# JanSpindler/NRC-HPM-Renderer

Hardware: AMD Instinct MI355X
Metric: Msamples/s + ms/frame at 1080p, 256^3 cloud (NRC path) (higher is better)
Workload: dtype f16 (fp16 MFMA operands, fp32 accumulate; fp32 integrator)

## Files before the change

nrc-hpm-renderer_amd/csrc/nrc_api.hip:

```cpp
#include <algorithm>
#include <array>
#include <chrono>
#include <cmath>
#include <cstdio>
#include <cstdlib>
#include <cstring>
#include <fstream>
#include <map>
#include <memory>
#include <mutex>
#include <random>
#include <string>
#include <thread>
#include <unordered_map>
#include <vector>

#include <dlfcn.h>
#include <rccl/rccl.h>

#include "nrc_integrator.hpp"
#include "nrc_mlp.hpp"
#include "nrc_checkpoint.hpp"
#include "nrc_occupancy.hpp"
#include "nrc_schedule.hpp"
// ... 317 lines not shown
    {
        if (owner_ == who) owner_ = nullptr;
        last_loss_event_ = nullptr;
    }

    void infer_all(const uint32_t* filter, hipStream_t s, bool skip_zero = false, const CompositeArgs* composite = nullptr,
                   const uint32_t* live_list = nullptr, const uint32_t* live_count = nullptr, hipEvent_t done = nullptr)
    {
        if (!initialised_) throw std::logic_error("SkyRenderer ERROR: InferAndTrain before Init");
        struct Tail {
            hipEvent_t e; hipStream_t s; bool armed = false;
            ~Tail() { if (armed) { try { finish_launch_tail(s); } catch (...) { launch_tail() = LaunchTail{}; } } else if (e) (void)hipEventRecord(e, s); }
        } tail{done, s};
        const bool one = infer_batches_.size() == 1;
        size_t last_batch = infer_batches_.size();
        for (size_t i = 0; i < infer_batches_.size(); i++)
            if (filter == nullptr || filter[i] != 0) last_batch = i;
        if (!one && filter == nullptr && live_list != nullptr && composite == nullptr && skip_zero && mlp_->encodes_in_kernel()) {
            if (done) { arm_launch_tail(done); tail.armed = true; }
            mlp_->infer(d_infer_in_, d_infer_out_, infer_count_, true, s, skip_zero, nullptr, live_list, live_count);
            return;
        }
        for (size_t i = 0; i < infer_batches_.size(); i++) {
            if (filter != nullptr && filter[i] == 0) continue;
            const auto& b = infer_batches_[i];
            if (done && i == last_batch) { arm_launch_tail(done); tail.armed = true; }
            CompositeArgs ca;
            if (composite) { ca = *composite; ca.q_base = b.first; }
            mlp_->infer(d_infer_in_ + (size_t)b.first * 5, d_infer_out_ + (size_t)b.first * 3, b.second, true, s, skip_zero, composite ? &ca : nullptr,
                        one ? live_list : nullptr, one ? live_count : nullptr);
        }
    }
    bool model_has_grid() const { return mlp_->has_grid(); }
    bool encodes_in_kernel() const { return mlp_->encodes_in_kernel(); }
    bool can_pre_encode(const void* who) const { return initialised_ && mlp_->can_pre_encode() && owner_ == who && owner_frames_ >= 2; }
    void pre_encode(const float* d_train_in, int parity, hipStream_t s)
    {
        pre_features_ = mlp_->pre_encode(d_train_in, train_batch_count_ * train_batch_size_, parity, s);
        pre_source_ = d_train_in;
    }
    bool wants_live_list() const { return infer_batches_.size() == 1 || mlp_->encodes_in_kernel(); }
    bool can_composite() const { return mlp_->can_composite(); }

    void train_all(hipStream_t st, hipEvent_t ev_infer_prev, hipEvent_t ev_infer_cur = nullptr, hipEvent_t done = nullptr)
    {
        if (!initialised_) throw std::logic_error("SkyRenderer ERROR: InferAndTrain before Init");
        poll_comm();
        for (uint32_t b = 0; b < train_batch_count_; b++) {
            const size_t o = (size_t)b * train_batch_size_;
            const bool vector_read = hook_ != nullptr || (comm_ != nullptr && !sparse_grid_);
            if (pre_source_ != d_train_in_) pre_features_ = nullptr;
            const void* ready = pre_features_ != nullptr ? (const void*)((const char*)pre_features_ + o * mlp_->enc_dims() * 2) : nullptr;
            mlp_->backward(d_train_in_ + o * 5, d_train_target_ + o * 3, train_batch_size_,
                           train_batch_size_ * loss_norm_factor_, st, vector_read, ready);
            if (comm_ || hook_) mlp_->guard_stale();
            if (comm_ && sparse_grid_) exchange_sparse(st);
            else if (comm_ && exchange_half_) exchange_half(st, mlp_->n_params());
            else if (comm_) Rccl::get().check(Rccl::get().all_reduce(mlp_->grad_ptr(), mlp_->grad_ptr(), (size_t)mlp_->n_params() + 2, ncclFloat,
                                                               ncclSum, comm_, st), "ncclAllReduce");
            if (hook_) {
                if (exchange_half_) round_grad_half(st, mlp_->n_params());
                hook_(hook_user_, mlp_->grad_ptr(), mlp_->n_params(), mlp_->loss_ptr(), (void*)st);
                if (exchange_half_) round_grad_half(st, mlp_->n_params(), true);
            }
            if (vector_read) mlp_->grad_vector_is_source();
            if (b == 0 && ev_infer_prev) NRC_HIP(hipStreamWaitEvent(st, ev_infer_prev, 0));
            if (b == 1 && ev_infer_cur) NRC_HIP(hipStreamWaitEvent(st, ev_infer_cur, 0));
            loss_pushed_++;
            const bool last = b + 1 == train_batch_count_;
            hipEvent_t after = (last && done) ? done : ev_loss_;
            LaunchTailScope tail(st, after);
            const bool published = mlp_->optimizer_step(st, loss_pushed_, d_loss_cell_);
            if (!published) {
                launch_last(k_publish_loss, dim3(1), dim3(1), 0u, st, (const float*)mlp_->loss_ptr(), loss_pushed_, d_loss_cell_);
                NRC_HIP(hipGetLastError());
            }
            tail.finish();
            last_loss_event_ = after;
        }
        if (train_batch_count_ == 0 && done) NRC_HIP(hipEventRecord(done, st));
        pre_features_ = nullptr;
    }

    void ensure_grid_lists(uint32_t n_lists)
    {
        const uint32_t cap = mlp_->grid_list_capacity(train_batch_size_);
        if (cap == grid_cap_ && n_lists <= grid_lists_) return;
        NRC_HIP(hipDeviceSynchronize());
        if (d_grid_send_) dev_free(d_grid_send_);
        if (d_grid_recv_) dev_free(d_grid_recv_);
        grid_cap_ = cap;
        grid_lists_ = n_lists;
        dev_alloc(&d_grid_send_, Mlp::grid_list_words(cap) * 4, "d_grid_send_");
        dev_alloc(&d_grid_recv_, Mlp::grid_list_words(cap) * 4 * n_lists, "d_grid_recv_");
    }
    void exchange_half(hipStream_t st, uint32_t n)
    {
        Rccl& r = Rccl::get();
        if (!r.group_start || !r.group_end) fail("librccl lacks ncclGroupStart / ncclGroupEnd");
        start_exchange_half(st, n);
        RcclGroup group(r);
        r.check(r.all_reduce(d_grad_half_, d_grad_half_, n, ncclHalf, ncclSum, comm_, st), "ncclAllReduce");
        r.check(r.all_reduce(mlp_->loss_ptr(), mlp_->loss_ptr(), 2, ncclFloat, ncclSum, comm_, st), "ncclAllReduce");
        group.end();
        finish_exchange_half(st, n);
    }
    void start_exchange_half(hipStream_t st, uint32_t n)
// ... 2417 lines not shown
```

nrc-hpm-renderer_amd/csrc/nrc_mlp.hip:

```cpp
#include "nrc_mlp.hpp"

#include <algorithm>
#include <cmath>
#include <cstdio>
#include <cstdlib>
#include <cstring>
#include <type_traits>

namespace nrc {

using half_t = _Float16;
using half8 = _Float16 __attribute__((ext_vector_type(8)));
using f32x16 = float __attribute__((ext_vector_type(16)));

namespace {

constexpr int ENC = 80;
constexpr int WIDTH = 64;
constexpr int KS0 = ENC / 16;
constexpr int KSH = WIDTH / 16;
constexpr int MT = WIDTH / 32;

__host__ __device__ inline int fmap80(int s, int h, int j)
{
// ... 1872 lines not shown
        }                                                                                                          \
    }
    NRC_WG_LOAD(a0, b0, 0)
    for (int s = 0; s < ksteps; s += 2 * U) {
        NRC_WG_LOAD(a1, b1, s + U)
        NRC_WG_MMA(a0, b0, s)
        NRC_WG_LOAD(a0, b0, s + 2 * U)
        NRC_WG_MMA(a1, b1, s + U)
    }
#undef NRC_WG_LOAD
#undef NRC_WG_MMA
#pragma unroll
    for (int t = 0; t < NTL; t++) {
        float* o = slab + T.param_off + 32u * (uint32_t)t + (uint32_t)r;
#pragma unroll
        for (int reg = 0; reg < 16; reg++) {
            const uint32_t row = (reg & 3) + 8 * (reg >> 2) + 4 * h;
            if (row < T.m_valid && bv[t]) o[(size_t)row * T.in_dim] = acc[t][reg];
        }
    }
}
#ifndef NRC_WGRAD2_MIN_WAVES
#define NRC_WGRAD2_MIN_WAVES 2
#endif
__global__ __launch_bounds__(WGRAD2_WAVES * 64, NRC_WGRAD2_MIN_WAVES) void k_wgrad2(const half_t* __restrict__ deltas, const half_t* __restrict__ acts, uint32_t n,
                                                             uint32_t chunk, uint32_t rows_d, uint32_t rows_a,
                                                             const WgradTask* __restrict__ tasks, int n_tasks, float* __restrict__ slabs,
                                                             uint32_t n_params)
{
    NRC_RAISE_WAVE_PRIORITY(1);
    const int lane = threadIdx.x & 63, wave = threadIdx.x >> 6;
    const int task = __builtin_amdgcn_readfirstlane((int)blockIdx.y * WGRAD2_WAVES + wave);
    if (task >= n_tasks) return;
    const WgradTask T = tasks[task];
    const uint32_t k0 = blockIdx.x * chunk;
    const uint32_t left = n - k0;
    const int ksteps = (int)((left < chunk ? left : chunk) >> 4);
    float* slab = slabs + (size_t)blockIdx.x * n_params;
    if constexpr (WGRAD2_NTL == 1) {
        wgrad_task<1>(T, deltas, acts, k0, ksteps, rows_d, rows_a, slab, lane);
    } else if constexpr (WGRAD2_NTL == 2) {
        if (T.n_tiles == 1) wgrad_task<1>(T, deltas, acts, k0, ksteps, rows_d, rows_a, slab, lane);
        else wgrad_task<2>(T, deltas, acts, k0, ksteps, rows_d, rows_a, slab, lane);
    } else {
        switch (T.n_tiles) {
        case 1: wgrad_task<1>(T, deltas, acts, k0, ksteps, rows_d, rows_a, slab, lane); break;
        case 2: wgrad_task<2>(T, deltas, acts, k0, ksteps, rows_d, rows_a, slab, lane); break;
        case 3: wgrad_task<3>(T, deltas, acts, k0, ksteps, rows_d, rows_a, slab, lane); break;
        default: wgrad_task<4>(T, deltas, acts, k0, ksteps, rows_d, rows_a, slab, lane); break;
        }
    }
}

template <class... Guard>
__global__ __launch_bounds__(256) void k_reduce_grads(const float* __restrict__ slabs, uint32_t n_chunks, uint32_t n_params,
                                                     float* __restrict__ grad, const float* __restrict__ loss_part,
                                                     uint32_t n_loss, float* __restrict__ loss, Guard... ga)
{
    NRC_RAISE_WAVE_PRIORITY(1);
    __shared__ float part[4][64];
    __shared__ float red[256];
    const uint32_t p = threadIdx.x & 63u, g = threadIdx.x >> 6;
    const uint32_t i = blockIdx.x * 64u + p;
    const uint32_t per = (n_chunks + 3u) / 4u;
    const uint32_t c0 = g * per, c1 = min(c0 + per, n_chunks);
    float s = 0.0f;
    if (i < n_params)
        for (uint32_t c = c0; c < c1; c++) s += slabs[(size_t)c * n_params + i];
    part[g][p] = s;
    __syncthreads();
    if (g == 0 && i < n_params) grad[i] = ((part[0][p] + part[1][p]) + part[2][p]) + part[3][p];
    if constexpr (sizeof...(Guard) != 0) guard_flag(g == 0 && i < n_params && guard_nonfinite(((part[0][p] + part[1][p]) + part[2][p]) + part[3][p]), ga...);
    if (blockIdx.x == 0) {
        float l = 0.0f;
        for (uint32_t k = threadIdx.x; k < n_loss; k += 256u) l += loss_part[k];
        red[threadIdx.x] = l;
        __syncthreads();
        for (int off = 128; off >= 1; off >>= 1) {
            if ((int)threadIdx.x < off) red[threadIdx.x] += red[threadIdx.x + off];
            __syncthreads();
        }
        if (threadIdx.x == 0) { loss[0] = red[0]; loss[1] = 0.0f; }
        if constexpr (sizeof...(Guard) != 0) guard_flag(threadIdx.x == 0 && guard_nonfinite(red[0]), ga...);
    }
}
__global__ __launch_bounds__(256) void k_guard_scan(const float* __restrict__ grad, uint32_t n, const float* __restrict__ loss, GuardArgs ga)
{
    NRC_RAISE_WAVE_PRIORITY(1);
    const uint32_t i = blockIdx.x * 256u + threadIdx.x;
    bool bad = i < n && guard_nonfinite(grad[i]);
    if (i == 0) bad = bad || guard_nonfinite(loss[0]);
    guard_flag(bad, ga);
}

struct AdamArgs {
    float lr_t, inv_loss_scale, ema_old, ema_new, ema_div;
};
#pragma clang fp contract(off)
__device__ __forceinline__ float ema_value(float e_old, float wi, const AdamArgs& a) { return (e_old * a.ema_old + wi * a.ema_new) / a.ema_div; }
__device__ __forceinline__ void adam_value(float& wi, float& mi, float& vi, float graw, bool matrix, const AdamArgs& a)
{
    const float b1 = 0.9f, b2 = 0.999f, eps = 1e-8f, l2 = 1e-8f;
    const float g = graw * a.inv_loss_scale + (matrix ? l2 * wi : 0.0f);
    const float m_new = b1 * mi + (1.0f - b1) * g;
    const float v_new = b2 * vi + (1.0f - b2) * (g * g);
    mi = m_new;
    vi = v_new;
    wi = wi - a.lr_t * m_new / (sqrtf(v_new) + eps);
}
__device__ __forceinline__ void sgd_value(float& wi, float graw, float lr, const AdamArgs& a)
{
    const float l2 = 1e-8f;
    const float g = graw * a.inv_loss_scale + l2 * wi;
    wi = wi - lr * g;
}
__device__ __forceinline__ void adam_ema_update(uint32_t i, float* __restrict__ w, float* __restrict__ ema, float* __restrict__ m,
                                                float* __restrict__ v, float graw, bool matrix, const AdamArgs& a, float* w_new,
                                                float* ema_new)
{
    float wi = w[i];
    if (!matrix && graw == 0.0f) {
        const float e = ema_value(ema[i], wi, a);
        ema[i] = e;
        *w_new = wi; *ema_new = e;
        return;
    }
    adam_value(wi, m[i], v[i], graw, matrix, a);
    w[i] = wi;
    const float e = ema_value(ema[i], wi, a);
    ema[i] = e;
    *w_new = wi; *ema_new = e;
}
__device__ __forceinline__ void sgd_ema_update(uint32_t i, float* __restrict__ w, float* __restrict__ ema, float graw, float lr,
                                               const AdamArgs& a, float* w_new, float* ema_new)
// ... 20 lines not shown
            return;
        }
    }
    float wn, en;
    adam_ema_update(i, w, ema, m, v, grad[i], i < n_matrix, a, &wn, &en);
}
template <class... Guard>
__global__ void k_sgd_ema(float* __restrict__ w, float* __restrict__ ema, const float* __restrict__ grad, uint32_t n, float lr,
                          AdamArgs a, Guard... ga)
{
    NRC_RAISE_WAVE_PRIORITY(1);
    const uint32_t i = blockIdx.x * blockDim.x + threadIdx.x;
    if (i >= n) return;
    if constexpr (sizeof...(Guard) != 0) {
        if (guard_bad(ga...)) {
            if (i == 0) guard_count(ga...);
            return;
        }
    }
    float wn, en;
    sgd_ema_update(i, w, ema, grad[i], lr, a, &wn, &en);
}

struct PackDst {
    const int32_t *fwd, *inf, *bwd;
    half_t *pk_fwd, *pk_inf, *pk_bwd;
};
template <bool SGD, class... Guard>
__global__ __launch_bounds__(256) void k_opt_pack(float* __restrict__ w, float* __restrict__ ema, float* __restrict__ m,
                                                 float* __restrict__ v, const float* __restrict__ grad, uint32_t n, float lr,
                                                 AdamArgs a, PackDst d, const float* __restrict__ loss, uint32_t loss_seq,
                                                 unsigned long long* __restrict__ loss_cell, Guard... ga)
{
    NRC_RAISE_WAVE_PRIORITY(1);
    const uint32_t i = blockIdx.x * blockDim.x + threadIdx.x;
    if (i == 0 && loss_cell != nullptr) {
        const unsigned long long bits = (unsigned long long)__builtin_bit_cast(uint32_t, loss[0]) | ((unsigned long long)loss_seq << 32);
        __hip_atomic_store(loss_cell, bits, __ATOMIC_RELAXED, __HIP_MEMORY_SCOPE_SYSTEM);
    }
    bool bad = false;
    if constexpr (sizeof...(Guard) != 0) {
        bad = guard_bad(ga...);
        if (i == 0 && bad) guard_count(ga...);
    }
    if (i >= n) return;
    float wn, en;
    if (sizeof...(Guard) != 0 && bad) { wn = w[i]; en = ema[i]; }
    else if (SGD) sgd_ema_update(i, w, ema, grad[i], lr, a, &wn, &en);
    else adam_ema_update(i, w, ema, m, v, grad[i], true, a, &wn, &en);
    const int32_t df = d.fwd[i], di = d.inf[i], db = d.bwd[i];
    if (df >= 0) d.pk_fwd[df] = (half_t)wn;
    if (di >= 0) d.pk_inf[di] = (half_t)en;
    if (db >= 0) d.pk_bwd[db] = (half_t)wn;
}

#pragma clang fp contract(off)
template <bool SGD, bool FROM16, class... Guard>
__global__ __launch_bounds__(256) void k_grid_opt2(float* __restrict__ w, float* __restrict__ ema, float* __restrict__ m,
                                                  float* __restrict__ v, const float* __restrict__ grad,
                                                  uint32_t* __restrict__ grad16, uint32_t n_matrix, uint32_t n_pairs, float lr,
                                                  AdamArgs a, uint32_t* __restrict__ t_train, uint32_t* __restrict__ t_ema, Guard... ga)
{
    NRC_RAISE_WAVE_PRIORITY(1);
    const uint32_t p = blockIdx.x * 256u + threadIdx.x;
    if (p >= n_pairs) return;
    const uint32_t e = 2u * p, i0 = n_matrix + 4u * p;
    float g[4];
    if (FROM16) {
        const uint2 word = *reinterpret_cast<const uint2*>(grad16 + e);
        const half2v h0 = __builtin_bit_cast(half2v, word.x), h1 = __builtin_bit_cast(half2v, word.y);
        g[0] = (float)h0[0]; g[1] = (float)h0[1]; g[2] = (float)h1[0]; g[3] = (float)h1[1];
        if ((word.x | word.y) != 0u) *reinterpret_cast<uint2*>(grad16 + e) = make_uint2(0u, 0u);
    } else {
        const float4 gv = *reinterpret_cast<const float4*>(grad + i0);
        g[0] = gv.x; g[1] = gv.y; g[2] = gv.z; g[3] = gv.w;
    }
    if constexpr (sizeof...(Guard) != 0) {
        if (guard_bad(ga...)) {
            const float4 ek = *reinterpret_cast<const float4*>(ema + i0);
            const float2v k0 = {ek.x, ek.y}, k1 = {ek.z, ek.w};
            *reinterpret_cast<uint2*>(t_ema + e) = make_uint2(__builtin_bit_cast(uint32_t, __builtin_convertvector(k0, half2v)),
                                                             __builtin_bit_cast(uint32_t, __builtin_convertvector(k1, half2v)));
            return;
        }
    }
    const float4 wv = *reinterpret_cast<const float4*>(w + i0), ev = *reinterpret_cast<const float4*>(ema + i0);
    float wi[4] = {wv.x, wv.y, wv.z, wv.w}, ei[4] = {ev.x, ev.y, ev.z, ev.w};
    const bool untouched = !SGD && g[0] == 0.0f && g[1] == 0.0f && g[2] == 0.0f && g[3] == 0.0f;
    if (!untouched) {
        if (SGD) {
#pragma unroll
            for (int k = 0; k < 4; k++) sgd_value(wi[k], g[k], lr, a);
        } else {
            const float4 mv = *reinterpret_cast<const float4*>(m + i0), vv = *reinterpret_cast<const float4*>(v + i0);
            float mi[4] = {mv.x, mv.y, mv.z, mv.w}, vi[4] = {vv.x, vv.y, vv.z, vv.w};
#pragma unroll
            for (int k = 0; k < 4; k++)
                if (g[k] != 0.0f) adam_value(wi[k], mi[k], vi[k], g[k], false, a);
            *reinterpret_cast<float4*>(m + i0) = make_float4(mi[0], mi[1], mi[2], mi[3]);
            *reinterpret_cast<float4*>(v + i0) = make_float4(vi[0], vi[1], vi[2], vi[3]);
        }
        *reinterpret_cast<float4*>(w + i0) = make_float4(wi[0], wi[1], wi[2], wi[3]);
        const float2v w0 = {wi[0], wi[1]}, w1 = {wi[2], wi[3]};
        *reinterpret_cast<uint2*>(t_train + e) = make_uint2(__builtin_bit_cast(uint32_t, __builtin_convertvector(w0, half2v)),
                                                           __builtin_bit_cast(uint32_t, __builtin_convertvector(w1, half2v)));
    }
// ... 181 lines not shown
        NRC_HIP(hipMemset(p, 0, sf.size() * 2));
    }
    fused_opt_ = !debug_switch("no_fused_opt");
    if (fused_opt_) {
        std::vector<int32_t> dst((size_t)3 * n_mlp_, -1);
        auto invert = [&](const int32_t* src, size_t n_slots, int32_t* out) {
            for (size_t j = 0; j < n_slots; j++) {
                if (src[j] < 0) continue;
                if ((uint32_t)src[j] >= n_mlp_ || out[src[j]] >= 0) { fused_opt_ = false; return; }
                out[src[j]] = (int32_t)j;
            }
        };
        std::vector<int32_t> si_host(sf.size());
        NRC_HIP(hipMemcpy(si_host.data(), d_src_inf_, sf.size() * 4, hipMemcpyDeviceToHost));
        invert(sf.data(), sf.size(), dst.data());
        if (fused_opt_) invert(si_host.data(), si_host.size(), dst.data() + n_mlp_);
        if (fused_opt_) invert(sb.data(), sb.size(), dst.data() + 2 * (size_t)n_mlp_);
        if (fused_opt_) {
            dev_alloc(&d_dst_, dst.size() * 4, "d_dst_");
            NRC_HIP(hipMemcpy(d_dst_, dst.data(), dst.size() * 4, hipMemcpyHostToDevice));
        }
    }
    dev_alloc(&d_pk_fwd_, sf.size() * 2, "d_pk_fwd_");
    dev_alloc(&d_pk_bwd_, sb.size() * 2, "d_pk_bwd_");
    if (hash_) {
        dev_alloc(&d_t16_train_, (size_t)n_grid_entries_ * 4, "d_t16_train_");
        for (auto& p : d_t16_ema_) dev_alloc(&p, (size_t)n_grid_entries_ * 4, "p");
        dev_alloc(&d_grad16_, (size_t)n_grid_entries_ * 4, "d_grad16_");
    }
    repack(nullptr);
    NRC_HIP(hipStreamSynchronize(nullptr));
}

Mlp::~Mlp()
{
    if (d_src_inf_ != d_src_fwd_ && d_src_inf_) dev_free(d_src_inf_);
    if (d_dst_) dev_free(d_dst_);
    void* ptrs[] = {d_w_, d_ema_, d_m_, d_v_, d_grad_, d_pk_infer_[0], d_pk_infer_[1], d_pk_fwd_, d_pk_bwd_, d_src_fwd_,
                    d_src_bwd_, d_acts_, d_deltas_, d_slabs_, d_loss_part_, d_tiles_, d_tasks_, d_feat_[0], d_feat_[1], d_feat_[2], d_feat_[3], d_feat_[4], d_t16_train_,
                    d_t16_ema_[0], d_t16_ema_[1], d_denc_, d_grad16_, d_grid_lists_, d_grid_counters_, d_grid_bin_entry0_, d_grid_fix_};
    for (void* p : ptrs)
        if (p) dev_free(p);
    if (d_guard_) dev_free(d_guard_);
    if (h_guard_) (void)hipHostFree(h_guard_);
}

float* Mlp::buffer(int which)
{
    switch (which) {
    case 0: return d_w_;
    case 1: return d_ema_;
    case 2: return d_m_;
    case 3: return d_v_;
    case 4: return d_grad_;
    default: fail("bad parameter buffer id");
    }
}

void Mlp::to_tcnn_layout(int which, const float* own, float* tcnn) const
{
    if (which < 0 || which > 4) fail("bad parameter buffer id");
    const size_t n_out = (size_t)3 * width_, head = n_mlp_ - n_out, dead = (size_t)13 * width_;
    std::memcpy(tcnn, own, (head + n_out) * sizeof(float));
    if (which < 4) std::memcpy(tcnn + n_mlp_, tcnn_dead_rows_[which].data(), dead * sizeof(float));
    else std::memset(tcnn + n_mlp_, 0, dead * sizeof(float));
    std::memcpy(tcnn + n_mlp_ + dead, own + n_mlp_, (size_t)(n_params_ - n_mlp_) * sizeof(float));
}

void Mlp::from_tcnn_layout(int which, const float* tcnn, float* own)
{
    if (which < 0 || which > 4) fail("bad parameter buffer id");
    const size_t dead = (size_t)13 * width_;
    std::memcpy(own, tcnn, (size_t)n_mlp_ * sizeof(float));
    if (which < 4) std::memcpy(tcnn_dead_rows_[which].data(), tcnn + n_mlp_, dead * sizeof(float));
    std::memcpy(own + n_mlp_, tcnn + n_mlp_ + dead, (size_t)(n_params_ - n_mlp_) * sizeof(float));
}

void Mlp::repack(hipStream_t s)
{
    const uint32_t nf = n_frag_fwd_ * 512, nb = n_frag_bwd_ * 512;
    const uint32_t nmax = nf > nb ? nf : nb;
    const int next = infer_set_ ^ 1;
    hipLaunchKernelGGL(k_pack, dim3(ceil_div(nmax, 256)), dim3(256), 0, s, d_w_, d_ema_, d_src_fwd_, d_src_inf_, nf, d_src_bwd_, nb,
                       (half_t*)d_pk_infer_[next], (half_t*)d_pk_fwd_, (half_t*)d_pk_bwd_);
    if (hash_)
        hipLaunchKernelGGL(k_pack_grid, dim3(ceil_div(n_grid_entries_, 256)), dim3(256), 0, s, d_w_ + n_mlp_, d_ema_ + n_mlp_,
                           (uint32_t*)d_t16_train_, (uint32_t*)d_t16_ema_[next], n_grid_entries_);
    NRC_HIP(hipGetLastError());
    infer_set_ = next;
}

void Mlp::launch_features(const float* d_in, uint32_t n, bool use_ema, int slot, hipStream_t s, bool skip_zero, const uint32_t* live_list,
                          const uint32_t* live_count)
{
    ensure_features(n, slot);
    half_t* feat = (half_t*)d_feat_[slot];
    if (!hash_) {
        launch_encode(cfg_.pos_id, cfg_.dir_id, s, d_in, feat, n, skip_zero);
        return;
    }
    HashLevels lv;
    for (uint32_t l = 0; l <= HG_LEVELS; l++) lv.off[l] = hg_off_[l];
    const uint32_t* tab = (const uint32_t*)(use_ema ? d_t16_ema_[infer_set_] : d_t16_train_);
    if (slot == 0 && live_list != nullptr && skip_zero) {
        const uint32_t n_slots = enc_dims_ / 2;
        dim3 g((uint32_t)num_cus() * 2u, n_slots);
        uint32_t xc = 0;
// ... 310 lines not shown
                info.insert(info.end(), {hg_off_[l] + b * GB_BIN, (uint32_t)(pairs + (size_t)b * grid_bin_cap_[l]), grid_bin_cap_[l], 0u});
            }
            pairs += (size_t)grid_bin_count_[l] * grid_bin_cap_[l];
            grid_bins_total_ += grid_bin_count_[l];
        }
        if (pairs > 0xffffffffull) fail("train batch too large for the table gradient's bin lists");
        if (grid_bins_total_ != 0u) {
            dev_alloc(&d_grid_lists_, pairs * 8, "d_grid_lists_");
            dev_alloc(&d_grid_counters_, (size_t)grid_bins_total_ * 4, "d_grid_counters_");
            NRC_HIP(hipMemset(d_grid_counters_, 0, (size_t)grid_bins_total_ * 4));
            dev_alloc(&d_grid_bin_entry0_, info.size() * 4, "d_grid_bin_info_");
            NRC_HIP(hipMemcpy(d_grid_bin_entry0_, info.data(), info.size() * 4, hipMemcpyHostToDevice));
        }
        if (!d_grid_fix_) {
            dev_alloc(&d_grid_fix_, (size_t)n_grid_entries_ * 16, "d_grid_fix_");
            NRC_HIP(hipMemset(d_grid_fix_, 0, (size_t)n_grid_entries_ * 16));
        }
    }
    dev_alloc(&d_loss_part_, (size_t)(n / 32) * 4, "d_loss_part_");
    ws_n_ = n;
    if (!d_tiles_) {
        std::vector<WgradTile> tiles;
        const uint32_t D = depth_;
        for (uint32_t l = 0; l <= D; l++) {
            const MlpLayer& L = layers_[l];
            const uint32_t a_rows = l == D ? D * kw_ : l * kw_;
            const uint32_t b_rows = l == 0 ? 0 : enc_dims_ + (l - 1) * kw_;
            for (uint32_t mt = 0; mt * 32 < L.out; mt++)
                for (uint32_t nt = 0; nt * 32 < L.in; nt++) {
                    WgradTile T;
                    T.a_row0 = a_rows + 32 * mt;
                    T.b_row0 = b_rows + 32 * nt;
                    T.m_valid = L.out - 32 * mt < 32 ? L.out - 32 * mt : 32;
                    T.n_valid = L.in - 32 * nt < 32 ? L.in - 32 * nt : 32;
                    T.param_off = L.off + 32 * mt * L.in + 32 * nt;
                    T.in_dim = L.in;
                    tiles.push_back(T);
                }
        }
        n_wgrad_tiles_ = (int)tiles.size();
        dev_alloc(&d_tiles_, tiles.size() * sizeof(WgradTile), "d_tiles_");
        NRC_HIP(hipMemcpy(d_tiles_, tiles.data(), tiles.size() * sizeof(WgradTile), hipMemcpyHostToDevice));
    }
}

const void* Mlp::pre_encode(const float* d_in, uint32_t n, int parity, hipStream_t s)
{
    if (!can_pre_encode()) fail("pre_encode: the model's encoding is trainable or computed inside its kernels");
    const int slot = 2 + (parity & 1);
    launch_features(d_in, n, false, slot, s, false);
    return d_feat_[slot];
}

void Mlp::backward(const float* d_in, const float* d_target, uint32_t n, uint32_t n_norm, hipStream_t s, bool widen_grid_grad, const void* features_ready)
{
    if (n == 0 || n % 32 != 0) fail("training batch must be a non-zero multiple of 32 samples");
    ensure_train_workspace(n);
    const uint32_t n_tiles = n / 32;
    constexpr int THREADS = 256;
    uint32_t blocks = ceil_div(n_tiles, THREADS / 64);
    if (fused_) {
        TrainArgs a;
        a.in = d_in;
        a.target = d_target;
        a.n = n;
        a.inv_n_total = (float)(1.0 / (3.0 * (double)n_norm));
        a.loss_id = loss_id_;
        a.acts = (half_t*)d_acts_;
        a.deltas = (half_t*)d_deltas_;
        a.loss_part = d_loss_part_;
        if (blocks > (uint32_t)num_cus()) blocks = (uint32_t)num_cus();
        const size_t lds = (size_t)std::max(n_frag_fwd_, n_frag_bwd_) * 1024;
        auto kernel = k_train_fwd_bwd_light<6, THREADS>;
        if (!attr_train_set_) {
            NRC_HIP(hipFuncSetAttribute(reinterpret_cast<const void*>(kernel), hipFuncAttributeMaxDynamicSharedMemorySize, (int)lds));
            attr_train_set_ = true;
        }
        hipLaunchKernelGGL(kernel, dim3(blocks), dim3(THREADS), lds, s, a, (const uint4*)d_pk_fwd_, (const uint4*)d_pk_bwd_);
    } else {
        if (features_ready == nullptr) launch_features(d_in, n, false, 1, s, false);
        if (hash_ && !grad16_clean_) NRC_HIP(hipMemsetAsync(d_grad16_, 0, (size_t)n_grid_entries_ * 4, s));
        grad16_clean_ = false;
        TrainArgsGen a;
        a.feat = features_ready != nullptr ? (const half_t*)features_ready : (const half_t*)d_feat_[1];
        a.target = d_target;
        a.n = n;
        a.inv_n_total = (float)(1.0 / (3.0 * (double)n_norm));
        a.loss_id = loss_id_;
        a.acts = (half_t*)d_acts_;
        a.deltas = (half_t*)d_deltas_;
        a.loss_part = d_loss_part_;
        a.depth = (int)depth_;
        a.ks0 = (int)enc_dims_ / 16;
        a.d_enc = hash_ ? (half_t*)d_denc_ : nullptr;
        const bool small = n_tiles <= (uint32_t)num_cus() * 8u;
        const uint32_t waves = small ? 4u : 8u;
        blocks = ceil_div(n_tiles, waves);
        const uint32_t cap = (uint32_t)num_cus() * 2u;
        if (blocks > cap) blocks = cap;
        const int mtg = (int)kw_ / 32, ksg = (int)kw_ / 16;
        const size_t lds = (size_t)2 * mtg * (ksg > 5 ? ksg : 5) * 1024 + waves * (KG_SCRATCH + (size_t)depth_ * 512);
        if (lds > 160 * 1024) fail("network too deep for the training kernel's LDS budget");
        if (!attr_train_set_) {
            const int cap_lds = 160 * 1024;
            NRC_HIP(hipFuncSetAttribute(reinterpret_cast<const void*>(&k_train_gen<32, 4>), hipFuncAttributeMaxDynamicSharedMemorySize, cap_lds));
            NRC_HIP(hipFuncSetAttribute(reinterpret_cast<const void*>(&k_train_gen<32, 8>), hipFuncAttributeMaxDynamicSharedMemorySize, cap_lds));
            NRC_HIP(hipFuncSetAttribute(reinterpret_cast<const void*>(&k_train_gen<64, 4>), hipFuncAttributeMaxDynamicSharedMemorySize, cap_lds));
            NRC_HIP(hipFuncSetAttribute(reinterpret_cast<const void*>(&k_train_gen<64, 8>), hipFuncAttributeMaxDynamicSharedMemorySize, cap_lds));
// ... 37 lines not shown
        } else if (kw_ == 64) {
            if (small) hipLaunchKernelGGL((k_train_gen<64, 4>), dim3(blocks), dim3(256), lds, s, a, fw, bw);
            else hipLaunchKernelGGL((k_train_gen<64, 8>), dim3(blocks), dim3(512), lds, s, a, fw, bw);
        } else {
            if (small) hipLaunchKernelGGL((k_train_gen<128, 4>), dim3(blocks), dim3(256), lds, s, a, fw, bw);
            else hipLaunchKernelGGL((k_train_gen<128, 8>), dim3(blocks), dim3(512), lds, s, a, fw, bw);
        }
        if (hash_) {
            HashLevels lv;
            for (uint32_t l = 0; l <= HG_LEVELS; l++) lv.off[l] = hg_off_[l];
            {
                GridBins gb;
                LooseRanges loose;
                loose.n = 0;
                uint32_t loose_chunks = 0;
                for (uint32_t l = 0; l < HG_LEVELS; l++) {
                    gb.first[l] = grid_bin_first_[l]; gb.count[l] = grid_bin_count_[l]; gb.cap[l] = grid_bin_cap_[l]; gb.list0[l] = grid_list0_[l];
                    if (grid_bin_count_[l] == 0u) {
                        loose.first[loose.n] = hg_off_[l];
                        loose.count[loose.n] = hg_off_[l + 1] - hg_off_[l];
                        loose_chunks += ceil_div(loose.count[loose.n], GB_BIN);
                        loose.n++;
                    }
                }
                for (uint32_t r = loose.n; r < HG_LEVELS; r++) loose.first[r] = loose.count[r] = 0u;
                if (!attr_gather_set_) {
                    NRC_HIP(hipFuncSetAttribute(reinterpret_cast<const void*>(&k_grid_gather), hipFuncAttributeMaxDynamicSharedMemorySize, (int)(GB_BIN * 16u)));
                    attr_gather_set_ = true;
                }
                const bool level_major = !xcd8_;
                hipLaunchKernelGGL(k_grid_scatter, level_major ? dim3(ceil_div(n, 256), HG_LEVELS) : dim3(ceil_div(n, 256) * HG_LEVELS, 1), dim3(256), 0, s, d_in, (const half_t*)d_denc_, (long long*)d_grid_fix_, n, lv,
                                   gb, (uint32_t*)d_grid_counters_, (uint2*)d_grid_lists_);
                hipLaunchKernelGGL(k_grid_gather, dim3(grid_bins_total_ + loose_chunks), dim3(NRC_GB_GATHER_THREADS), GB_BIN * 16u, s, (uint32_t*)d_grad16_,
                                   (const uint4*)d_grid_bin_entry0_, grid_bins_total_, (uint32_t*)d_grid_counters_, (const uint2*)d_grid_lists_, (long long*)d_grid_fix_, loose);
            }
            grid16_valid_ = fused_opt_;
            if (widen_grid_grad || !fused_opt_)
                hipLaunchKernelGGL(k_grid_grad_f32, dim3(ceil_div(n_grid_entries_, 256)), dim3(256), 0, s, (const uint32_t*)d_grad16_,
                                   d_grad_ + n_mlp_, n_grid_entries_);
        }
    }
    NRC_HIP(hipGetLastError());
    const uint32_t chunk = wgrad_chunk(n);
    const uint32_t n_chunks = ceil_div(n, chunk);
    if (wgrad_old_)
        hipLaunchKernelGGL(k_wgrad, dim3(n_chunks), dim3(WGRAD_WAVES * 64), 0, s, (const half_t*)d_deltas_, (const half_t*)d_acts_, n,
                           depth_ * kw_ + 8, enc_dims_ + depth_ * kw_, (const WgradTile*)d_tiles_, n_wgrad_tiles_, d_slabs_,
                           n_mlp_);
    else
        hipLaunchKernelGGL(k_wgrad2, dim3(n_chunks, ceil_div((uint32_t)n_wgrad_tasks_, (uint32_t)WGRAD2_WAVES)), dim3(WGRAD2_WAVES * 64), 0, s,
                           (const half_t*)d_deltas_, (const half_t*)d_acts_, n, chunk, depth_ * kw_ + 8, enc_dims_ + depth_ * kw_,
                           (const WgradTask*)d_tasks_, n_wgrad_tasks_, d_slabs_, n_mlp_);
    NRC_HIP(hipGetLastError());
    auto reduce = [&](auto... ga) {
        hipLaunchKernelGGL(k_reduce_grads<decltype(ga)...>, dim3(ceil_div(n_mlp_, 64)), dim3(256), 0, s, d_slabs_, n_chunks, n_mlp_,
                           d_grad_, d_loss_part_, n_tiles, d_loss_, ga...);
    };
    if (guard_on_) reduce(guard_scan_args());
    else reduce();
    NRC_HIP(hipGetLastError());
}

void Mlp::set_guard(bool on)
{
    if (on && !d_guard_) {
        dev_alloc((void**)&d_guard_, 4 * sizeof(uint32_t), "d_guard_");
        NRC_HIP(hipMemset(d_guard_, 0, 4 * sizeof(uint32_t)));
        NRC_HIP(hipHostMalloc((void**)&h_guard_, sizeof(unsigned long long), hipHostMallocMapped));
        *h_guard_ = 0ull;
        NRC_HIP(hipHostGetDevicePointer((void**)&d_guard_cell_, h_guard_, 0));
    }
    guard_on_ = on;
    guard_scanned_ = false;
}

GuardArgs Mlp::guard_scan_args()
{
    if (++guard_stamp_ == 0u) guard_stamp_ = 1u;
    guard_scanned_ = true;
    return GuardArgs{d_guard_, d_guard_cell_, guard_stamp_, 0u};
}

void Mlp::guard_stats(uint32_t* skipped, uint32_t* last_step) const
{
    const unsigned long long bits = h_guard_ ? __atomic_load_n(h_guard_, __ATOMIC_ACQUIRE) : 0ull;
    *skipped = (uint32_t)bits;
    *last_step = (uint32_t)(bits >> 32);
}

uint32_t Mlp::grid_list_capacity(uint32_t n) const
{
    const unsigned long long touched = (unsigned long long)n * HG_LEVELS * 8ull;
    return (uint32_t)std::min<unsigned long long>(touched, n_grid_entries_);
}

void Mlp::grid_grad_pack(uint32_t* d_list, uint32_t cap, hipStream_t s)
{
    if (!hash_) fail("grid_grad_pack: this model has no trainable encoding");
    NRC_HIP(hipMemsetAsync(d_list, 0xff, grid_list_words(cap) * 4, s));
    NRC_HIP(hipMemsetAsync(d_list, 0, 8, s));
    hipLaunchKernelGGL(k_grid_pack, dim3(ceil_div(n_grid_entries_, 4096)), dim3(256), 0, s, (const uint32_t*)d_grad16_,
                       n_grid_entries_, d_list, cap);
    NRC_HIP(hipGetLastError());
}

void Mlp::grid_grad_apply(const uint32_t* d_lists, uint32_t n_lists, uint32_t cap, hipStream_t s)
{
    if (!hash_) fail("grid_grad_apply: this model has no trainable encoding");
    grid16_valid_ = false;
    NRC_HIP(hipMemsetAsync(d_grad_ + n_mlp_, 0, (size_t)n_grid_entries_ * 8, s));
    for (uint32_t r = 0; r < n_lists; r++)
        hipLaunchKernelGGL(k_grid_apply, dim3(ceil_div(cap, 256)), dim3(256), 0, s, d_lists + (size_t)r * grid_list_words(cap), cap,
                           d_grad_ + n_mlp_, n_grid_entries_);
    NRC_HIP(hipGetLastError());
}

static AdamArgs adam_args_of(const nrc_config& cfg, uint32_t step)
{
    const double b1 = 0.9, b2 = 0.999;
    const double t = (double)step;
    const double d = (double)cfg.ema_decay;
    AdamArgs a;
    a.lr_t = cfg.learning_rate * (float)(std::sqrt(1.0 - std::pow(b2, t)) / (1.0 - std::pow(b1, t)));
    a.inv_loss_scale = 1.0f / Mlp::kLossScale;
    a.ema_old = (float)(d * (1.0 - std::pow(d, t - 1.0)));
    a.ema_new = (float)(1.0 - d);
    a.ema_div = (float)(1.0 - std::pow(d, t));
    return a;
}

template <class F>
static void with_flag(bool on, F&& f)
{
    if (on) f(std::true_type{});
    else f(std::false_type{});
}

bool Mlp::optimizer_step(hipStream_t s, uint32_t loss_seq, unsigned long long* loss_cell)
{
    step += 1;
    const AdamArgs a = adam_args_of(cfg_, step);
    if (guard_on_) {
        if (!guard_scanned_) {
            hipLaunchKernelGGL(k_guard_scan, dim3(ceil_div(n_mlp_, 256)), dim3(256), 0, s, (const float*)d_grad_, n_mlp_, (const float*)d_loss_,
                               guard_scan_args());
            NRC_HIP(hipGetLastError());
        }
        guard_scanned_ = false;
    }
    const float lr = cfg_.learning_rate;
    const dim3 b(256);
    auto enqueue = [&](auto... ga) {
        if (!fused_opt_) {
            if (sgd_) hipLaunchKernelGGL(k_sgd_ema<decltype(ga)...>, dim3(ceil_div(n_params_, 256)), b, 0, s, d_w_, d_ema_, d_grad_, n_params_, lr, a, ga...);
            else hipLaunchKernelGGL(k_adam_ema<decltype(ga)...>, dim3(ceil_div(n_params_, 256)), b, 0, s, d_w_, d_ema_, d_m_, d_v_, d_grad_, n_params_, n_mlp_, a, ga...);
            NRC_HIP(hipGetLastError());
            repack(s);
            return false;
        }
        const int next = infer_set_ ^ 1;
        const PackDst d{d_dst_, d_dst_ + n_mlp_, d_dst_ + 2 * (size_t)n_mlp_, (half_t*)d_pk_fwd_, (half_t*)d_pk_infer_[next], (half_t*)d_pk_bwd_};
        const float* loss = d_loss_;
        with_flag(sgd_, [&](auto sgd) {
            constexpr bool SGD = decltype(sgd)::value;
            const auto pack = k_opt_pack<SGD, decltype(ga)...>;
            auto launch = [&](auto... args) {
                if (hash_) hipLaunchKernelGGL(pack, dim3(ceil_div(n_mlp_, 256)), b, 0, s, args...);
                else launch_last(pack, dim3(ceil_div(n_mlp_, 256)), b, 0u, s, args...);
            };
            launch(d_w_, d_ema_, d_m_, d_v_, d_grad_, n_mlp_, lr, a, d, loss, loss_seq, loss_cell, ga...);
            if (!hash_) return;
            uint32_t *tt = (uint32_t*)d_t16_train_, *te = (uint32_t*)d_t16_ema_[next], *g16 = (uint32_t*)d_grad16_;
            const uint32_t np = n_grid_entries_ / 2u;
            if (grid16_valid_) grad16_clean_ = true;
            with_flag(grid16_valid_, [&](auto from16) {
                launch_last(k_grid_opt2<SGD, decltype(from16)::value, decltype(ga)...>, dim3(ceil_div(np, 256)), b, 0u, s, d_w_, d_ema_, d_m_, d_v_, d_grad_,
                            g16, n_mlp_, np, lr, a, tt, te, ga...);
            });
        });
        NRC_HIP(hipGetLastError());
        infer_set_ = next;
        return loss_cell != nullptr;
    };
    return guard_on_ ? enqueue(GuardArgs{d_guard_, d_guard_cell_, guard_stamp_, step}) : enqueue();
}

}
```

nrc-hpm-renderer_amd/csrc/nrc_mlp.hpp:

```cpp
#pragma once
#include <vector>

#include "nrc_common.hpp"

namespace nrc {

struct MlpLayer {
    uint32_t out, in;
    uint32_t off;
};

struct CompositeArgs {
    const float* primary;
    const float* info;
    float* framebuffer;
    uint32_t w, h, show_nrc, q_base;
    float blend_factor;
};

struct GuardArgs {
    uint32_t* words = nullptr;
    unsigned long long* host_cell = nullptr;
    uint32_t stamp = 0, step = 0;
};
#if defined(__HIPCC__)
__device__ __forceinline__ bool guard_nonfinite(float x) { return (__builtin_bit_cast(uint32_t, x) & 0x7f800000u) == 0x7f800000u; }
__device__ __forceinline__ void guard_flag(bool bad, const GuardArgs& ga)
{
    const unsigned long long found = __ballot(bad);
    if (found != 0ull && (threadIdx.x & 63u) == (uint32_t)(__ffsll((long long)found) - 1)) ga.words[0] = ga.stamp;
}
__device__ __forceinline__ bool guard_bad(const GuardArgs& ga) { return ga.words[0] == ga.stamp; }
__device__ __forceinline__ void guard_count(const GuardArgs& ga)
{
    const uint32_t skipped = ga.words[1] + 1u;
    ga.words[1] = skipped;
    ga.words[2] = ga.step;
    __hip_atomic_store(ga.host_cell, (unsigned long long)skipped | ((unsigned long long)ga.step << 32), __ATOMIC_RELAXED, __HIP_MEMORY_SCOPE_SYSTEM);
}
#endif

void mlp_set_wave_priority_raise(int on);

class Mlp {
public:
    explicit Mlp(const nrc_config& cfg);
    ~Mlp();
    Mlp(const Mlp&) = delete;
    Mlp& operator=(const Mlp&) = delete;

    static constexpr int kInferSlot = 0, kSideSlot = 4;
    void infer(const float* d_in, float* d_out, uint32_t n, bool use_ema, hipStream_t s, bool skip_zero_queries = false,
               const CompositeArgs* composite = nullptr, const uint32_t* live_list = nullptr, const uint32_t* live_count = nullptr,
               int feat_slot = kInferSlot);
    void reserve_side_slot(uint32_t n) { if (!encodes_in_kernel()) ensure_features(n, kSideSlot); }
    bool can_composite() const { return fused_; }
    bool encodes_in_kernel() const { return fused_ || enc80_generic_; }
    void backward(const float* d_in, const float* d_target, uint32_t n, uint32_t n_norm, hipStream_t s, bool widen_grid_grad = true,
                  const void* features_ready = nullptr);
    bool can_pre_encode() const { return !fused_ && !hash_; }
    const void* pre_encode(const float* d_in, uint32_t n, int parity, hipStream_t s);
    void grad_vector_is_source() { grid16_valid_ = false; }
    bool optimizer_step(hipStream_t s, uint32_t loss_seq = 0, unsigned long long* loss_cell = nullptr);
    void repack(hipStream_t s);

    uint32_t n_params() const { return n_params_; }
    uint32_t enc_dims() const { return enc_dims_; }
    float* grad_ptr() { return d_grad_; }
    float* loss_ptr() { return d_loss_; }
    float* buffer(int which);
    uint32_t tcnn_param_count() const { return n_params_ + 13u * width_; }
    void to_tcnn_layout(int which, const float* own, float* tcnn) const;
    void from_tcnn_layout(int which, const float* tcnn, float* own);
    bool has_grid() const { return hash_; }
    uint32_t n_mlp_params() const { return n_mlp_; }
    uint32_t grid_entries() const { return n_grid_entries_; }
    uint32_t grid_list_capacity(uint32_t n_batch) const;
    static size_t grid_list_words(uint32_t cap) { return 2 + 2 * (size_t)cap; }
    void grid_grad_pack(uint32_t* d_list, uint32_t cap, hipStream_t s);
    void grid_grad_apply(const uint32_t* d_lists, uint32_t n_lists, uint32_t cap, hipStream_t s);
    uint32_t step = 0;
    static constexpr float kLossScale = 128.0f;

    void set_guard(bool on);
    bool guard_on() const { return guard_on_; }
    void guard_stale() { guard_scanned_ = false; }
    void grad_written_from_outside() { grad_vector_is_source(); guard_stale(); }
    GuardArgs guard_scan_args();
    void guard_stats(uint32_t* skipped, uint32_t* last_step) const;

private:
    bool guard_on_ = false, guard_scanned_ = false;
    uint32_t guard_stamp_ = 0;
    uint32_t* d_guard_ = nullptr;
    unsigned long long* h_guard_ = nullptr;
    unsigned long long* d_guard_cell_ = nullptr;
    int num_cus();
    int num_cus_ = 0;
    bool attr_infer_set_ = false, attr_infer4_set_ = false, attr_train_set_ = false, attr_train2_set_ = false;
    void ensure_train_workspace(uint32_t n);
    void ensure_features(uint32_t n, int slot);
    void launch_features(const float* d_in, uint32_t n, bool use_ema, int slot, hipStream_t s, bool skip_zero, const uint32_t* live_list = nullptr,
                         const uint32_t* live_count = nullptr);
#ifdef NRC_DIAG
    void infer_diagnostic(int abl, uint32_t blocks, size_t lds, hipStream_t s, const float* d_in, float* d_out, uint32_t n,
                          const void* image);
#endif

    nrc_config cfg_;
    uint32_t width_, depth_, enc_dims_, n_params_;
    uint32_t kw_ = 0;
    uint32_t loss_id_;
    bool sgd_ = false;
    bool fused_ = false;
    std::vector<MlpLayer> layers_;
    void* d_feat_[5] = {nullptr, nullptr, nullptr, nullptr, nullptr};
    uint32_t feat_n_[5] = {0, 0, 0, 0, 0};
    int infer_set_ = 0;
    uint32_t n_mlp_ = 0;
    bool hash_ = false;
    bool xcd8_ = true;
    uint32_t hg_off_[17] = {0};
    uint32_t n_grid_entries_ = 0;
    void *d_t16_train_ = nullptr, *d_t16_ema_[2] = {nullptr, nullptr};
    void* d_denc_ = nullptr;
    void* d_grad16_ = nullptr;
    void *d_grid_lists_ = nullptr, *d_grid_counters_ = nullptr, *d_grid_bin_entry0_ = nullptr, *d_grid_fix_ = nullptr;
    uint32_t grid_bin_first_[16] = {}, grid_bin_count_[16] = {}, grid_bin_cap_[16] = {}, grid_list0_[16] = {}, grid_bins_total_ = 0;
    bool attr_gather_set_ = false;

    float *d_w_ = nullptr, *d_ema_ = nullptr, *d_m_ = nullptr, *d_v_ = nullptr, *d_grad_ = nullptr, *d_loss_ = nullptr;
    std::vector<float> tcnn_dead_rows_[4];
    void *d_pk_infer_[2] = {nullptr, nullptr}, *d_pk_fwd_ = nullptr, *d_pk_bwd_ = nullptr;
    int32_t *d_src_fwd_ = nullptr, *d_src_bwd_ = nullptr;
    int32_t* d_dst_ = nullptr;
    bool fused_opt_ = false;
    bool grad16_clean_ = false;
    bool grid16_valid_ = false;
    int32_t* d_src_inf_ = nullptr;
    bool enc80_generic_ = false;
    uint32_t n_frag_fwd_ = 0, n_frag_bwd_ = 0;

    uint32_t ws_n_ = 0;
    void* d_acts_ = nullptr;
    void* d_deltas_ = nullptr;
    float* d_slabs_ = nullptr;
    float* d_loss_part_ = nullptr;
    void* d_tiles_ = nullptr;
    int n_wgrad_tiles_ = 0;
    void* d_tasks_ = nullptr;
    int n_wgrad_tasks_ = 0;
    bool wgrad_old_ = false;
    void build_wgrad_tasks();
    uint32_t wgrad_chunk(uint32_t n);
};

}
```

Before: 8965.

## Defer gradient slab reduction and fuse it into the optimizer pack kernel

The backward pass now records a pending reduction instead of always launching k_reduce_grads. When no comm, hook or guard is active and the fused optimizer is used, the slab reduction, loss fold, Adam/SGD update, EMA and fp16 repack all run in one new kernel. This removes a kernel launch and a round trip of the grad vector through global memory. Accessors like grad_ptr and loss_ptr force the reduction first, so other paths stay correct. The cost is added lazy-state bookkeeping and a wider grid (64 params per block) for the optimizer step.

```diff
diff --git a/nrc-hpm-renderer_amd/csrc/nrc_api.hip b/nrc-hpm-renderer_amd/csrc/nrc_api.hip
--- a/nrc-hpm-renderer_amd/csrc/nrc_api.hip
+++ b/nrc-hpm-renderer_amd/csrc/nrc_api.hip
@@ -393,7 +393,7 @@
             if (pre_source_ != d_train_in_) pre_features_ = nullptr;
             const void* ready = pre_features_ != nullptr ? (const void*)((const char*)pre_features_ + o * mlp_->enc_dims() * 2) : nullptr;
             mlp_->backward(d_train_in_ + o * 5, d_train_target_ + o * 3, train_batch_size_,
-                           train_batch_size_ * loss_norm_factor_, st, vector_read, ready);
+                           train_batch_size_ * loss_norm_factor_, st, vector_read, ready, comm_ == nullptr && hook_ == nullptr);
             if (comm_ || hook_) mlp_->guard_stale();
             if (comm_ && sparse_grid_) exchange_sparse(st);
             else if (comm_ && exchange_half_) exchange_half(st, mlp_->n_params());
diff --git a/nrc-hpm-renderer_amd/csrc/nrc_mlp.hip b/nrc-hpm-renderer_amd/csrc/nrc_mlp.hip
--- a/nrc-hpm-renderer_amd/csrc/nrc_mlp.hip
+++ b/nrc-hpm-renderer_amd/csrc/nrc_mlp.hip
@@ -1948,14 +1948,8 @@
     }
 }
 
-template <class... Guard>
-__global__ __launch_bounds__(256) void k_reduce_grads(const float* __restrict__ slabs, uint32_t n_chunks, uint32_t n_params,
-                                                     float* __restrict__ grad, const float* __restrict__ loss_part,
-                                                     uint32_t n_loss, float* __restrict__ loss, Guard... ga)
-{
-    NRC_RAISE_WAVE_PRIORITY(1);
-    __shared__ float part[4][64];
-    __shared__ float red[256];
+__device__ __forceinline__ void slab_partials(const float* __restrict__ slabs, uint32_t n_chunks, uint32_t n_params, float (*part)[64])
+{
     const uint32_t p = threadIdx.x & 63u, g = threadIdx.x >> 6;
     const uint32_t i = blockIdx.x * 64u + p;
     const uint32_t per = (n_chunks + 3u) / 4u;
@@ -1965,17 +1959,34 @@
         for (uint32_t c = c0; c < c1; c++) s += slabs[(size_t)c * n_params + i];
     part[g][p] = s;
     __syncthreads();
-    if (g == 0 && i < n_params) grad[i] = ((part[0][p] + part[1][p]) + part[2][p]) + part[3][p];
-    if constexpr (sizeof...(Guard) != 0) guard_flag(g == 0 && i < n_params && guard_nonfinite(((part[0][p] + part[1][p]) + part[2][p]) + part[3][p]), ga...);
+}
+__device__ __forceinline__ float slab_sum(const float (*part)[64], uint32_t p) { return ((part[0][p] + part[1][p]) + part[2][p]) + part[3][p]; }
+__device__ __forceinline__ void fold_loss(const float* __restrict__ loss_part, uint32_t n_loss, float* red)
+{
+    float l = 0.0f;
+    for (uint32_t k = threadIdx.x; k < n_loss; k += 256u) l += loss_part[k];
+    red[threadIdx.x] = l;
+    __syncthreads();
+    for (int off = 128; off >= 1; off >>= 1) {
+        if ((int)threadIdx.x < off) red[threadIdx.x] += red[threadIdx.x + off];
+        __syncthreads();
+    }
+}
+template <class... Guard>
+__global__ __launch_bounds__(256) void k_reduce_grads(const float* __restrict__ slabs, uint32_t n_chunks, uint32_t n_params,
+                                                     float* __restrict__ grad, const float* __restrict__ loss_part,
+                                                     uint32_t n_loss, float* __restrict__ loss, Guard... ga)
+{
+    NRC_RAISE_WAVE_PRIORITY(1);
+    __shared__ float part[4][64];
+    __shared__ float red[256];
+    const uint32_t p = threadIdx.x & 63u, g = threadIdx.x >> 6;
+    const uint32_t i = blockIdx.x * 64u + p;
+    slab_partials(slabs, n_chunks, n_params, part);
+    if (g == 0 && i < n_params) grad[i] = slab_sum(part, p);
+    if constexpr (sizeof...(Guard) != 0) guard_flag(g == 0 && i < n_params && guard_nonfinite(slab_sum(part, p)), ga...);
     if (blockIdx.x == 0) {
-        float l = 0.0f;
-        for (uint32_t k = threadIdx.x; k < n_loss; k += 256u) l += loss_part[k];
-        red[threadIdx.x] = l;
-        __syncthreads();
-        for (int off = 128; off >= 1; off >>= 1) {
-            if ((int)threadIdx.x < off) red[threadIdx.x] += red[threadIdx.x + off];
-            __syncthreads();
-        }
+        fold_loss(loss_part, n_loss, red);
         if (threadIdx.x == 0) { loss[0] = red[0]; loss[1] = 0.0f; }
         if constexpr (sizeof...(Guard) != 0) guard_flag(threadIdx.x == 0 && guard_nonfinite(red[0]), ga...);
     }
@@ -2102,6 +2113,42 @@
     if (df >= 0) d.pk_fwd[df] = (half_t)wn;
     if (di >= 0) d.pk_inf[di] = (half_t)en;
     if (db >= 0) d.pk_bwd[db] = (half_t)wn;
+}
+
+template <bool SGD>
+__global__ __launch_bounds__(256) void k_reduce_opt_pack(const float* __restrict__ slabs, uint32_t n_chunks, const float* __restrict__ loss_part,
+                                                        uint32_t n_loss, float* __restrict__ w, float* __restrict__ ema, float* __restrict__ m,
+                                                        float* __restrict__ v, float* __restrict__ grad, uint32_t n, float lr, AdamArgs a,
+                                                        PackDst d, float* __restrict__ loss, uint32_t loss_seq,
+                                                        unsigned long long* __restrict__ loss_cell)
+{
+    NRC_RAISE_WAVE_PRIORITY(1);
+    __shared__ float part[4][64];
+    __shared__ float red[256];
+    const uint32_t p = threadIdx.x & 63u, g = threadIdx.x >> 6;
+    const uint32_t i = blockIdx.x * 64u + p;
+    slab_partials(slabs, n_chunks, n, part);
+    if (g == 0 && i < n) {
+        const float graw = slab_sum(part, p);
+        grad[i] = graw;
+        float wn, en;
+        if (SGD) sgd_ema_update(i, w, ema, graw, lr, a, &wn, &en);
+        else adam_ema_update(i, w, ema, m, v, graw, true, a, &wn, &en);
+        const int32_t df = d.fwd[i], di = d.inf[i], db = d.bwd[i];
+        if (df >= 0) d.pk_fwd[df] = (half_t)wn;
+        if (di >= 0) d.pk_inf[di] = (half_t)en;
+        if (db >= 0) d.pk_bwd[db] = (half_t)wn;
+    }
+    if (blockIdx.x == 0) {
+        fold_loss(loss_part, n_loss, red);
+        if (threadIdx.x == 0) {
+            loss[0] = red[0]; loss[1] = 0.0f;
+            if (loss_cell != nullptr) {
+                const unsigned long long bits = (unsigned long long)__builtin_bit_cast(uint32_t, red[0]) | ((unsigned long long)loss_seq << 32);
+                __hip_atomic_store(loss_cell, bits, __ATOMIC_RELAXED, __HIP_MEMORY_SCOPE_SYSTEM);
+            }
+        }
+    }
 }
 
 #pragma clang fp contract(off)
@@ -2389,7 +2436,7 @@
     case 1: return d_ema_;
     case 2: return d_m_;
     case 3: return d_v_;
-    case 4: return d_grad_;
+    case 4: return grad_ptr();
     default: fail("bad parameter buffer id");
     }
 }
@@ -2806,8 +2853,10 @@
     return d_feat_[slot];
 }
 
-void Mlp::backward(const float* d_in, const float* d_target, uint32_t n, uint32_t n_norm, hipStream_t s, bool widen_grid_grad, const void* features_ready)
-{
+void Mlp::backward(const float* d_in, const float* d_target, uint32_t n, uint32_t n_norm, hipStream_t s, bool widen_grid_grad, const void* features_ready,
+                   bool defer_reduce)
+{
+    reduce_now();
     if (n == 0 || n % 32 != 0) fail("training batch must be a non-zero multiple of 32 samples");
     ensure_train_workspace(n);
     const uint32_t n_tiles = n / 32;
@@ -2951,9 +3000,18 @@
                            (const half_t*)d_deltas_, (const half_t*)d_acts_, n, chunk, depth_ * kw_ + 8, enc_dims_ + depth_ * kw_,
                            (const WgradTask*)d_tasks_, n_wgrad_tasks_, d_slabs_, n_mlp_);
     NRC_HIP(hipGetLastError());
+    unreduced_ = Unreduced{true, n_chunks, n_tiles, s};
+    if (!(defer_reduce && fused_opt_ && !guard_on_)) reduce_now();
+}
+
+void Mlp::reduce_now()
+{
+    if (!unreduced_.pending) return;
+    const Unreduced u = unreduced_;
+    unreduced_.pending = false;
     auto reduce = [&](auto... ga) {
-        hipLaunchKernelGGL(k_reduce_grads<decltype(ga)...>, dim3(ceil_div(n_mlp_, 64)), dim3(256), 0, s, d_slabs_, n_chunks, n_mlp_,
-                           d_grad_, d_loss_part_, n_tiles, d_loss_, ga...);
+        hipLaunchKernelGGL(k_reduce_grads<decltype(ga)...>, dim3(ceil_div(n_mlp_, 64)), dim3(256), 0, u.stream, d_slabs_, u.n_chunks, n_mlp_,
+                           d_grad_, d_loss_part_, u.n_loss, d_loss_, ga...);
     };
     if (guard_on_) reduce(guard_scan_args());
     else reduce();
@@ -2969,6 +3027,7 @@
         *h_guard_ = 0ull;
         NRC_HIP(hipHostGetDevicePointer((void**)&d_guard_cell_, h_guard_, 0));
     }
+    reduce_now();
     guard_on_ = on;
     guard_scanned_ = false;
 }
@@ -3049,6 +3108,8 @@
     }
     const float lr = cfg_.learning_rate;
     const dim3 b(256);
+    const bool reduce_here = unreduced_.pending && fused_opt_ && !guard_on_;
+    if (!reduce_here) reduce_now();
     auto enqueue = [&](auto... ga) {
         if (!fused_opt_) {
             if (sgd_) hipLaunchKernelGGL(k_sgd_ema<decltype(ga)...>, dim3(ceil_div(n_params_, 256)), b, 0, s, d_w_, d_ema_, d_grad_, n_params_, lr, a, ga...);
@@ -3062,12 +3123,18 @@
         const float* loss = d_loss_;
         with_flag(sgd_, [&](auto sgd) {
             constexpr bool SGD = decltype(sgd)::value;
-            const auto pack = k_opt_pack<SGD, decltype(ga)...>;
-            auto launch = [&](auto... args) {
-                if (hash_) hipLaunchKernelGGL(pack, dim3(ceil_div(n_mlp_, 256)), b, 0, s, args...);
-                else launch_last(pack, dim3(ceil_div(n_mlp_, 256)), b, 0u, s, args...);
+            auto launch = [&](auto kernel, dim3 grid, auto... args) {
+                if (hash_) hipLaunchKernelGGL(kernel, grid, b, 0, s, args...);
+                else launch_last(kernel, grid, b, 0u, s, args...);
             };
-            launch(d_w_, d_ema_, d_m_, d_v_, d_grad_, n_mlp_, lr, a, d, loss, loss_seq, loss_cell, ga...);
+            if (reduce_here) {
+                launch(k_reduce_opt_pack<SGD>, dim3(ceil_div(n_mlp_, 64)), (const float*)d_slabs_, unreduced_.n_chunks, (const float*)d_loss_part_, unreduced_.n_loss,
+                       d_w_, d_ema_, d_m_, d_v_, d_grad_, n_mlp_, lr, a, d, d_loss_, loss_seq, loss_cell);
+                unreduced_.pending = false;
+            } else {
+                launch(k_opt_pack<SGD, decltype(ga)...>, dim3(ceil_div(n_mlp_, 256)), d_w_, d_ema_, d_m_, d_v_, (const float*)d_grad_, n_mlp_, lr, a, d, loss, loss_seq,
+                       loss_cell, ga...);
+            }
             if (!hash_) return;
             uint32_t *tt = (uint32_t*)d_t16_train_, *te = (uint32_t*)d_t16_ema_[next], *g16 = (uint32_t*)d_grad16_;
             const uint32_t np = n_grid_entries_ / 2u;
diff --git a/nrc-hpm-renderer_amd/csrc/nrc_mlp.hpp b/nrc-hpm-renderer_amd/csrc/nrc_mlp.hpp
--- a/nrc-hpm-renderer_amd/csrc/nrc_mlp.hpp
+++ b/nrc-hpm-renderer_amd/csrc/nrc_mlp.hpp
@@ -57,17 +57,17 @@
     bool can_composite() const { return fused_; }
     bool encodes_in_kernel() const { return fused_ || enc80_generic_; }
     void backward(const float* d_in, const float* d_target, uint32_t n, uint32_t n_norm, hipStream_t s, bool widen_grid_grad = true,
-                  const void* features_ready = nullptr);
+                  const void* features_ready = nullptr, bool defer_reduce = false);
     bool can_pre_encode() const { return !fused_ && !hash_; }
     const void* pre_encode(const float* d_in, uint32_t n, int parity, hipStream_t s);
-    void grad_vector_is_source() { grid16_valid_ = false; }
+    void grad_vector_is_source() { reduce_now(); grid16_valid_ = false; }
     bool optimizer_step(hipStream_t s, uint32_t loss_seq = 0, unsigned long long* loss_cell = nullptr);
     void repack(hipStream_t s);
 
     uint32_t n_params() const { return n_params_; }
     uint32_t enc_dims() const { return enc_dims_; }
-    float* grad_ptr() { return d_grad_; }
-    float* loss_ptr() { return d_loss_; }
+    float* grad_ptr() { reduce_now(); return d_grad_; }
+    float* loss_ptr() { reduce_now(); return d_loss_; }
     float* buffer(int which);
     uint32_t tcnn_param_count() const { return n_params_ + 13u * width_; }
     void to_tcnn_layout(int which, const float* own, float* tcnn) const;
@@ -146,6 +146,12 @@
     void* d_deltas_ = nullptr;
     float* d_slabs_ = nullptr;
     float* d_loss_part_ = nullptr;
+    struct Unreduced {
+        bool pending = false;
+        uint32_t n_chunks = 0, n_loss = 0;
+        hipStream_t stream = nullptr;
+    } unreduced_;
+    void reduce_now();
     void* d_tiles_ = nullptr;
     int n_wgrad_tiles_ = 0;
     void* d_tasks_ = nullptr;
```

Result: slower. 8865 (-1.1%).
